# cemlyn007/ale-libtorch-ppo

Measured on AMD Instinct MI355X. Metric: env steps/sec (whole node), Breakout 84x84x4, higher is better.
Workload: dtype bf16

## Files before the change

### ale-libtorch-ppo_amd/csrc/gemm_launch.hip

```cpp
#include "common.hpp"
#include "gemm.hpp"
#include "gemm_pipe.hpp"
#include <algorithm>
#include <cstdlib>

namespace aleppo {

static int tune(const char *name, int dflt) {
  const char *e = std::getenv(name);
  return e ? std::atoi(e) : dflt;
}
static inline dim3 grid2(long M, int BM, long N, int BN, int Z = 1) {
  return dim3((unsigned)((M + BM - 1) / BM), (unsigned)((N + BN - 1) / BN), (unsigned)Z);
}

template <class T, bool IDX = false>
static void conv1_fwd_t(hipStream_t s, const uint32_t *obs, SampleMap map, const void *W1, const float *b1, void *a1,
                        long ns) {
  if constexpr (!IDX)
    if (map.idx)
      return conv1_fwd_t<T, true>(s, obs, map, W1, b1, a1, ns);
  using AL = ConvGatherLoader<T, uint8_t, 400, 20, 4, 84, 4, 8, IDX>;
  using BL = DenseLoader<T>;
  using EP = EpiBiasAct<T, true>;
  const long M = ns * 400;
  typename AL::P ap{reinterpret_cast<const uint8_t *>(obs), map.TP, map.s1 * 4, map.s0 * 4, map.base * 4, map.n0, map.idx};
  typename BL::P bp{static_cast<const T *>(W1), 256, 0};
  typename EP::P ep{static_cast<T *>(a1), b1, 32, 1.0f / 255.0f};
  hipLaunchKernelGGL((gemm_nt_kernel<T, AL, BL, EP, 128, 32, 4, 1>), grid2(M, 128, 32, 32), dim3(256), 0, s, ap, bp,
                     ep, (int)M, 32, 256);
}
template <class T>
static void conv2_fwd_t(hipStream_t s, const void *a1, const void *W2, const float *b2, void *a2, long ns) {
  using AL = ConvGatherLoader<T, T, 81, 9, 2, 20, 32, 4>;
  using BL = DenseLoader<T>;
  using EP = EpiBiasAct<T, true>;
  const long M = ns * 81;
  typename AL::P ap{static_cast<const T *>(a1), 1, 400 * 32, 0, 0, 0};
  typename BL::P bp{static_cast<const T *>(W2), 512, 0};
  typename EP::P ep{static_cast<T *>(a2), b2, 64, 1.0f};
  hipLaunchKernelGGL((gemm_nt_kernel<T, AL, BL, EP, 128, 64, 2, 2>), grid2(M, 128, 64, 64), dim3(256), 0, s, ap, bp,
                     ep, (int)M, 64, 512);
}
template <class T>
static void conv3_fwd_t(hipStream_t s, const void *a2, const void *W3, const float *b3, void *a3, long ns) {
  using AL = ConvGatherLoader<T, T, 49, 7, 1, 9, 64, 3>;
  using BL = DenseLoader<T>;
  using EP = EpiBiasAct<T, true>;
  const long M = ns * 49;
  typename AL::P ap{static_cast<const T *>(a2), 1, 81 * 64, 0, 0, 0};
  typename BL::P bp{static_cast<const T *>(W3), 576, 0};
  typename EP::P ep{static_cast<T *>(a3), b3, 64, 1.0f};
  hipLaunchKernelGGL((gemm_nt_kernel<T, AL, BL, EP, 128, 64, 2, 2>), grid2(M, 128, 64, 64), dim3(256), 0, s, ap, bp,
                     ep, (int)M, 64, 576);
}

static int pipe_cus() {
  static int n = 0;
  if (!n) {
    int dev = 0;
    hipDeviceProp_t p;
    if (hipGetDevice(&dev) == hipSuccess && hipGetDeviceProperties(&p, dev) == hipSuccess)
      n = p.multiProcessorCount;
    if (n <= 0)
      n = 256;
  }
  return n;
}
template <int MODE, int NST> static void launch_pipe(hipStream_t s, const PipeParams &P) {
  static bool once = false;
  constexpr size_t sm = gemm_pipe_smem<MODE, NST>();
  static_assert(sm <= 160 * 1024, "LDS budget");
  if (!once) {
    (void)hipFuncSetAttribute(reinterpret_cast<const void *>(gemm_pipe_kernel<MODE, NST>),
                              hipFuncAttributeMaxDynamicSharedMemorySize, (int)sm);
    once = true;
  }
  const int cus = pipe_cus() / 8 * 8, rounds = (P.njobs + cus - 1) / cus;
  const int grid = P.njobs >= cus / 4 ? std::min(cus, ((P.njobs + rounds - 1) / rounds + 7) / 8 * 8) : std::min(P.njobs, cus);
  hipLaunchKernelGGL((gemm_pipe_kernel<MODE, NST>), dim3(grid), dim3(PIPE_THREADS), sm, s, P);
}
static bool fc_dma() {
  static const bool v = tune("ALEPPO_FC_DMA", 1) != 0;
  return v;
}
static bool tn_xcd() {
  static const bool v = tune("ALEPPO_TN_XCD", 1) != 0;
  return v;
}
static bool use_pipe() { return tuning().fc_pipe; }
static int fc_fwd_pipe(hipStream_t s, const void *a3, const void *Wfc, const float *bfc, float *h, long ns, int H,
                       int max_parts) {
  const int tm = (int)((ns + 127) / 128), tn = (H + 127) / 128, tiles = tm * tn, cus = pipe_cus();
  int best = 1;
  double best_t = 1e30;
  for (int sp = 1; sp <= max_parts; ++sp) {
    const double t = (double)((tiles * sp + cus - 1) / cus) / sp + 0.02 * sp;
    if (t < best_t - 1e-9) {
      best_t = t;
      best = sp;
    }
  }
  PipeParams P{};
  P.A = static_cast<const bf16 *>(a3);
  P.lda = FC_IN;
  P.B = static_cast<const bf16 *>(Wfc);
  P.ldb = FC_IN;
  P.M = (int)ns;
  P.N = H;
  P.tiles_m = tm;
  P.tiles_n = tn;
  P.nstages = FC_IN / 64;
  P.splits = best;
  P.njobs = tiles * best;
  P.out_f32 = h;
  P.bias = bfc;
  launch_pipe<0, 4>(s, P);
  return best;
}
static void fc_dgrad_pipe(hipStream_t s, const void *dh, const void *WfcT, const void *a3, void *dz3, long ns, int H) {
  PipeParams P{};
  P.A = static_cast<const bf16 *>(dh);
  P.lda = H;
  P.B = static_cast<const bf16 *>(WfcT);
  P.ldb = H;
  P.M = (int)ns;
  P.N = FC_IN;
  P.tiles_m = (int)((ns + 127) / 128);
  P.tiles_n = (FC_IN + 127) / 128;
  P.nstages = H / 64;
  P.splits = 1;
  P.njobs = P.tiles_m * P.tiles_n;
  P.out_bf16 = static_cast<bf16 *>(dz3);
  P.gate = static_cast<const bf16 *>(a3);
  launch_pipe<1, 4>(s, P);
}
template <class T>
static void fc_fwd_t(hipStream_t s, const void *a3, const void *Wfc, const float *bfc, float *h, long ns, int H) {
  using AL = DenseLoader<T>;
  using BL = DenseLoader<T>;
  using EP = EpiBiasAct<float, false>;
  typename AL::P ap{static_cast<const T *>(a3), FC_IN, 0};
  typename BL::P bp{static_cast<const T *>(Wfc), FC_IN, 0};
  typename EP::P ep{h, bfc, H, 1.0f};
  if (ns <= 256)
    hipLaunchKernelGGL((gemm_nt_kernel<T, AL, BL, EP, 32, 32, 2, 2>), grid2(ns, 32, H, 32), dim3(256), 0, s, ap, bp,
                       ep, (int)ns, H, FC_IN);
  else if (fc_dma() && FC_IN % Atom<T>::KT == 0) {
    static const int v = tune("ALEPPO_FC_FWD_TILE", 1);
    const T *a = static_cast<const T *>(a3), *b = static_cast<const T *>(Wfc);
    if (v == 3 && FC_IN % (2 * Atom<T>::KT) == 0)
      hipLaunchKernelGGL((gemm_nt_dma_kernel<T, EP, 64, 64, 2, 2, 16>), grid2(ns, 64, H, 64), dim3(256), 0, s, a, FC_IN,
                         b, FC_IN, ep, (int)ns, H, FC_IN);
    else if (v == 4 && FC_IN % (2 * Atom<T>::KT) == 0)
      hipLaunchKernelGGL((gemm_nt_dma_kernel<T, EP, 128, 64, 2, 2, 16>), grid2(ns, 128, H, 64), dim3(256), 0, s, a,
                         FC_IN, b, FC_IN, ep, (int)ns, H, FC_IN);
    else if (v == 1)
      hipLaunchKernelGGL((gemm_nt_dma_kernel<T, EP, 64, 64, 2, 2>), grid2(ns, 64, H, 64), dim3(256), 0, s, a, FC_IN, b,
                         FC_IN, ep, (int)ns, H, FC_IN);
    else if (v == 2)
      hipLaunchKernelGGL((gemm_nt_dma_kernel<T, EP, 128, 128, 2, 2>), grid2(ns, 128, H, 128), dim3(256), 0, s, a,
                         FC_IN, b, FC_IN, ep, (int)ns, H, FC_IN);
    else
      hipLaunchKernelGGL((gemm_nt_dma_kernel<T, EP, 128, 64, 2, 2>), grid2(ns, 128, H, 64), dim3(256), 0, s, a, FC_IN,
                         b, FC_IN, ep, (int)ns, H, FC_IN);
  } else {
    static const int v = tune("ALEPPO_FC_FWD_TILE", 1);
    if (v == 1)
      hipLaunchKernelGGL((gemm_nt_kernel<T, AL, BL, EP, 64, 64, 2, 2>), grid2(ns, 64, H, 64), dim3(256), 0, s, ap, bp,
                         ep, (int)ns, H, FC_IN);
    else if (v == 2)
      hipLaunchKernelGGL((gemm_nt_kernel<T, AL, BL, EP, 128, 128, 2, 2>), grid2(ns, 128, H, 128), dim3(256), 0, s, ap,
                         bp, ep, (int)ns, H, FC_IN);
    else if (v == 3)
      hipLaunchKernelGGL((gemm_nt_kernel<T, AL, BL, EP, 64, 128, 2, 2>), grid2(ns, 64, H, 128), dim3(256), 0, s, ap,
                         bp, ep, (int)ns, H, FC_IN);
    else
      hipLaunchKernelGGL((gemm_nt_kernel<T, AL, BL, EP, 128, 64, 2, 2>), grid2(ns, 128, H, 64), dim3(256), 0, s, ap,
                         bp, ep, (int)ns, H, FC_IN);
  }
}

template <class T> static void fc_fwd_splitk_t(hipStream_t s, const void *a3, const void *Wfc, float *hpart, long ns, int H) {
  using AL = DenseLoader<T>;
  using BL = DenseLoader<T>;
  using EP = EpiPartial;
  constexpr int KC = FC_IN / FC_SPLITS;
  typename AL::P ap{static_cast<const T *>(a3), FC_IN, KC};
  typename BL::P bp{static_cast<const T *>(Wfc), FC_IN, KC};
  typename EP::P ep{hpart, H, ns * (long)H};
  hipLaunchKernelGGL((gemm_nt_kernel<T, AL, BL, EP, 32, 32, 2, 2>), grid2(ns, 32, H, 32, FC_SPLITS), dim3(256), 0, s,
                     ap, bp, ep, (int)ns, H, KC);
}
__global__ __launch_bounds__(256) void fc_act_kernel(const bf16 *__restrict__ a3, const bf16 *__restrict__ Wfc,
                                                     float *__restrict__ hpart, int M, int N) {
  constexpr int KC = FC_IN / FC_SPLITS, KS = KC / 32, VPR = KC / 8;
  constexpr int ROWV = VPR + 1;
  constexpr int NV = 32 * VPR / 256;
  __shared__ u32x4 sA[32 * ROWV], sB[32 * ROWV];
  const int tid = threadIdx.x, lane = tid & 63, wave = tid >> 6, fr = lane & 15, fg = lane >> 4;
  const int wm = wave >> 1, wn = wave & 1, z = blockIdx.z;
  const int m0 = blockIdx.x * 32, n0 = blockIdx.y * 32;
  u32x4 ra[NV], rb[NV];
#pragma unroll
  for (int i = 0; i < NV; ++i) {
    const int v = tid + 256 * i, r = v / VPR, c = v - r * VPR;
    ra[i] = *reinterpret_cast<const u32x4 *>(a3 + (long)min(m0 + r, M - 1) * FC_IN + z * KC + c * 8);
    rb[i] = *reinterpret_cast<const u32x4 *>(Wfc + (long)min(n0 + r, N - 1) * FC_IN + z * KC + c * 8);
  }
#pragma unroll
  for (int i = 0; i < NV; ++i) {
    const int v = tid + 256 * i, r = v / VPR, c = v - r * VPR;
    sA[r * ROWV + c] = ra[i];
    sB[r * ROWV + c] = rb[i];
  }
  __syncthreads();
  f32x4 acc = {0.f, 0.f, 0.f, 0.f};
#pragma unroll
  for (int ks = 0; ks < KS; ++ks)
    Atom<bf16>::mma(sA[(wm * 16 + fr) * ROWV + ks * 4 + fg], sB[(wn * 16 + fr) * ROWV + ks * 4 + fg], acc);
  float *out = hpart + (long)z * M * N;
  const int nn = n0 + wn * 16 + fr;
#pragma unroll
  for (int r = 0; r < 4; ++r) {
    const int mm = m0 + wm * 16 + fg * 4 + r;
    if (mm < M && nn < N)
      out[(long)mm * N + nn] = acc[r];
  }
}
void fc_fwd_splitk(hipStream_t s, int prec, const void *a3, const void *Wfc, float *hpart, long ns, int H) {
  static const bool latency_form = tune("ALEPPO_FC_ACT_LATENCY", 1) != 0;
  if (prec == ALEPPO_BF16 && latency_form)
    hipLaunchKernelGGL(fc_act_kernel, grid2(ns, 32, H, 32, FC_SPLITS), dim3(256), 0, s, static_cast<const bf16 *>(a3),
                       static_cast<const bf16 *>(Wfc), hpart, (int)ns, H);
  else if (prec == ALEPPO_BF16)
    fc_fwd_splitk_t<bf16>(s, a3, Wfc, hpart, ns, H);
  else
    fc_fwd_splitk_t<float>(s, a3, Wfc, hpart, ns, H);
}

template <class T>
static void fc_dgrad_t(hipStream_t s, const void *dh, const void *WfcT, const void *a3, void *dz3, long ns, int H) {
  using AL = DenseLoader<T>;
  using BL = DenseLoader<T>;
  using EP = EpiReluMask<T, 0>;
  typename AL::P ap{static_cast<const T *>(dh), H, 0};
  typename BL::P bp{static_cast<const T *>(WfcT), H, 0};
  typename EP::P ep{static_cast<T *>(dz3), static_cast<const T *>(a3), FC_IN, 0};
  static const int v = tune("ALEPPO_FC_DGRAD_TILE", 1);
  if (fc_dma() && H % Atom<T>::KT == 0) {
    const T *a = static_cast<const T *>(dh), *b = static_cast<const T *>(WfcT);
    if (v == 3)
      hipLaunchKernelGGL((gemm_nt_dma_kernel<T, EP, 64, 64, 2, 2, 16>), grid2(ns, 64, FC_IN, 64), dim3(256), 0, s, a, H,
                         b, H, ep, (int)ns, FC_IN, H);
    else if (v == 4)
      hipLaunchKernelGGL((gemm_nt_dma_kernel<T, EP, 128, 64, 2, 2, 16>), grid2(ns, 128, FC_IN, 64), dim3(256), 0, s, a,
                         H, b, H, ep, (int)ns, FC_IN, H);
    else if (v == 2)
      hipLaunchKernelGGL((gemm_nt_dma_kernel<T, EP, 128, 128, 2, 2>), grid2(ns, 128, FC_IN, 128), dim3(256), 0, s, a,
                         H, b, H, ep, (int)ns, FC_IN, H);
    else if (v == 0)
      hipLaunchKernelGGL((gemm_nt_dma_kernel<T, EP, 128, 64, 2, 2>), grid2(ns, 128, FC_IN, 64), dim3(256), 0, s, a, H,
                         b, H, ep, (int)ns, FC_IN, H);
    else
      hipLaunchKernelGGL((gemm_nt_dma_kernel<T, EP, 64, 64, 2, 2>), grid2(ns, 64, FC_IN, 64), dim3(256), 0, s, a, H, b,
                         H, ep, (int)ns, FC_IN, H);
    return;
  }
  if (v == 1)
    hipLaunchKernelGGL((gemm_nt_kernel<T, AL, BL, EP, 64, 64, 2, 2>), grid2(ns, 64, FC_IN, 64), dim3(256), 0, s, ap, bp,
                       ep, (int)ns, FC_IN, H);
  else if (v == 2)
    hipLaunchKernelGGL((gemm_nt_kernel<T, AL, BL, EP, 128, 128, 2, 2>), grid2(ns, 128, FC_IN, 128), dim3(256), 0, s,
                       ap, bp, ep, (int)ns, FC_IN, H);
  else
    hipLaunchKernelGGL((gemm_nt_kernel<T, AL, BL, EP, 128, 64, 2, 2>), grid2(ns, 128, FC_IN, 64), dim3(256), 0, s, ap,
                       bp, ep, (int)ns, FC_IN, H);
}
template <class T>
static void conv3_dgrad_t(hipStream_t s, const void *dz3, const void *W3d, const void *a2, void *dz2, long ns) {
  using AL = DgradGatherLoader<T, 9, 9, 7, 7, 64, 3>;
  using BL = DenseLoader<T>;
  using EP = EpiReluMask<T, 0>;
  const long M = ns * 81;
  typename AL::P ap{static_cast<const T *>(dz3)};
  typename BL::P bp{static_cast<const T *>(W3d), 576, 0};
  typename EP::P ep{static_cast<T *>(dz2), static_cast<const T *>(a2), 64, 0};
  hipLaunchKernelGGL((gemm_nt_kernel<T, AL, BL, EP, 128, 64, 2, 2>), grid2(M, 128, 64, 64), dim3(256), 0, s, ap, bp,
                     ep, (int)M, 64, 576);
}
template <class T>
static void conv2_dgrad_t(hipStream_t s, const void *dz2, const void *W2d, const void *a1, void *dz1, long ns) {
  using AL = DgradGatherLoader<T, 10, 10, 9, 9, 64, 2>;
  using BL = DenseLoader<T>;
  using EP = EpiReluMask<T, 1>;
  const long M = ns * 100;
  typename AL::P ap{static_cast<const T *>(dz2)};
  typename BL::P bp{static_cast<const T *>(W2d), 256, 32 * 256};
  typename EP::P ep{static_cast<T *>(dz1), static_cast<const T *>(a1), 32, 0};
  hipLaunchKernelGGL((gemm_nt_kernel<T, AL, BL, EP, 128, 32, 4, 1>), grid2(M, 128, 32, 32, 4), dim3(256), 0, s, ap,
                     bp, ep, (int)M, 32, 256);
}

static inline int pick_slices(long Ktot, int KP, int tiles_mn, int maxS) {
  long S = 512 / tiles_mn;
  const long cap = Ktot / (2L * KP);
  if (S > cap)
    S = cap;
  if (S > maxS)
    S = maxS;
  if (S < 1)
    S = 1;
  return (int)S;
}
static inline int chunk_for(long Ktot, int S, int KP) {
  long c = (Ktot + S - 1) / S;
  c = (c + KP - 1) / KP * KP;
  return (int)c;
}

static int fc_wgrad_split_max() { return tune("ALEPPO_FC_WGRAD_SPLIT", 2); }

template <class T> static int fc_wgrad_t(hipStream_t s, const void *dh, const void *a3, float *sw, float *sb, long ns, int H) {
  using AL = DenseLoader<T>;
  using BL = DenseLoader<T>;
  constexpr int KP = Atom<T>::KT;
  static const int v = tune("ALEPPO_FC_WGRAD_TILE", 0);
  static const int smax = fc_wgrad_split_max();
  const int S = (int)std::max<long>(1, std::min<long>(std::min(smax, MAXS_FC), ns / (4 * KP)));
  const int kc = chunk_for(ns, S, KP);
  typename AL::P ap{static_cast<const T *>(dh), H, 0};
  typename BL::P bp{static_cast<const T *>(a3), FC_IN, 0};
  auto swz = [&](const dim3 &g) { return ((g.x * g.y * S) % 8 == 0 && tn_xcd()) ? (int)(g.x | (g.y << 12)) : 0; };
  auto grid = [&](const dim3 &g, int xsw) { return xsw ? dim3(g.x * g.y * S) : dim3(g.x, g.y, S); };
  if (v == 1) {
    const dim3 g = grid2(H, 64, FC_IN, 64);
    const int xsw = swz(g);
    hipLaunchKernelGGL((gemm_tn_kernel<T, AL, BL, 64, 64, 2, 2, true>), grid(g, xsw), dim3(256), 0, s, ap, bp, sw,
                       sb, H, FC_IN, (int)ns, kc, 1.0f, xsw);
  } else if (v == 2) {
    const dim3 g = grid2(H, 128, FC_IN, 64);
    const int xsw = swz(g);
    hipLaunchKernelGGL((gemm_tn_kernel<T, AL, BL, 128, 64, 2, 2, true>), grid(g, xsw), dim3(256), 0, s, ap, bp,
                       sw, sb, H, FC_IN, (int)ns, kc, 1.0f, xsw);
  } else {
    const dim3 g = grid2(H, 64, FC_IN, 128);
    const int xsw = swz(g);
    hipLaunchKernelGGL((gemm_tn_kernel<T, AL, BL, 64, 128, 2, 2, true>), grid(g, xsw), dim3(256), 0, s, ap, bp,
                       sw, sb, H, FC_IN, (int)ns, kc, 1.0f, xsw);
  }
  return S;
}
template <class T> static int conv3_wgrad_t(hipStream_t s, const void *dz3, const void *a2, float *sw, float *sb, long ns) {
  using AL = DenseLoader<T>;
  using BL = ConvGatherLoader<T, T, 49, 7, 1, 9, 64, 3>;
  constexpr int KP = Atom<T>::KT;
  const long K = ns * 49;
  const dim3 g = grid2(64, 64, 576, 64);
  const int S = pick_slices(K, KP, g.x * g.y, MAXS_C3);
  const int kc = chunk_for(K, S, KP);
  typename AL::P ap{static_cast<const T *>(dz3), 64, 0};
  typename BL::P bp{static_cast<const T *>(a2), 1, 81 * 64, 0, 0, 0};
  hipLaunchKernelGGL((gemm_tn_kernel<T, AL, BL, 64, 64, 2, 2, true>), dim3(g.x, g.y, S), dim3(256), 0, s, ap, bp, sw,
                     sb, 64, 576, (int)K, kc, 1.0f, 0);
  return S;
}
template <class T> static int conv2_wgrad_t(hipStream_t s, const void *dz2, const void *a1, float *sw, float *sb, long ns) {
  using AL = DenseLoader<T>;
  using BL = ConvGatherLoader<T, T, 81, 9, 2, 20, 32, 4>;
  constexpr int KP = Atom<T>::KT;
  const long K = ns * 81;
  const dim3 g = grid2(64, 64, 512, 128);
  const int S = pick_slices(K, KP, g.x * g.y, MAXS_C2);
  const int kc = chunk_for(K, S, KP);
  typename AL::P ap{static_cast<const T *>(dz2), 64, 0};
  typename BL::P bp{static_cast<const T *>(a1), 1, 400 * 32, 0, 0, 0};
  hipLaunchKernelGGL((gemm_tn_kernel<T, AL, BL, 64, 128, 2, 2, true>), dim3(g.x, g.y, S), dim3(256), 0, s, ap, bp, sw,
                     sb, 64, 512, (int)K, kc, 1.0f, 0);
  return S;
}
template <class T, bool IDX = false>
static int conv1_wgrad_t(hipStream_t s, const void *dz1, const uint32_t *obs, SampleMap map, float *sw, float *sb,
                         long ns) {
  if constexpr (!IDX)
    if (map.idx)
      return conv1_wgrad_t<T, true>(s, dz1, obs, map, sw, sb, ns);
  using AL = DenseLoader<T>;
  using BL = ConvGatherLoader<T, uint8_t, 400, 20, 4, 84, 4, 8, IDX>;
  constexpr int KP = Atom<T>::KT;
  const long K = ns * 400;
  const dim3 g = grid2(32, 32, 256, 128);
  const int S = pick_slices(K, KP, g.x * g.y, MAXS_C1);
  const int kc = chunk_for(K, S, KP);
  typename AL::P ap{static_cast<const T *>(dz1), 32, 0};
  typename BL::P bp{reinterpret_cast<const uint8_t *>(obs), map.TP, map.s1 * 4, map.s0 * 4, map.base * 4, map.n0, map.idx};
  hipLaunchKernelGGL((gemm_tn_kernel<T, AL, BL, 32, 128, 1, 4, true>), dim3(g.x, g.y, S), dim3(256), 0, s, ap, bp, sw,
                     sb, 32, 256, (int)K, kc, 1.0f / 255.0f, 0);
  return S;
}

#define DISPATCH(prec, call_f32, call_bf16)                                                                            \
  do {                                                                                                                 \
    if ((prec) == ALEPPO_BF16) {                                                                                       \
      call_bf16;                                                                                                       \
    } else {                                                                                                           \
      call_f32;                                                                                                        \
    }                                                                                                                  \
  } while (0)

void conv1_fwd(hipStream_t s, int prec, const uint32_t *obs, SampleMap map, const void *W1, const float *b1, void *a1,
               long ns) {
  if (prec == ALEPPO_BF16 && use_patch_kernels())
    return patch_conv1_fwd(s, obs, map, W1, b1, a1, ns);
  DISPATCH(prec, conv1_fwd_t<float>(s, obs, map, W1, b1, a1, ns), conv1_fwd_t<bf16>(s, obs, map, W1, b1, a1, ns));
}
void conv2_fwd(hipStream_t s, int prec, const void *a1, const void *W2, const float *b2, void *a2, long ns) {
  if (prec == ALEPPO_BF16 && use_patch_kernels())
    return patch_conv2_fwd(s, a1, W2, b2, a2, ns);
  DISPATCH(prec, conv2_fwd_t<float>(s, a1, W2, b2, a2, ns), conv2_fwd_t<bf16>(s, a1, W2, b2, a2, ns));
}
void conv3_fwd(hipStream_t s, int prec, const void *a2, const void *W3, const float *b3, void *a3, long ns) {
  if (prec == ALEPPO_BF16 && use_patch_kernels())
    return patch_conv3_fwd(s, a2, W3, b3, a3, ns);
  DISPATCH(prec, conv3_fwd_t<float>(s, a2, W3, b3, a3, ns), conv3_fwd_t<bf16>(s, a2, W3, b3, a3, ns));
}
int fc_fwd(hipStream_t s, int prec, const void *a3, const void *Wfc, const float *bfc, float *h, long ns, int H,
           int max_parts) {
  if (prec == ALEPPO_BF16 && ns > 256 && H % 64 == 0 && H >= 64 && use_pipe())
    return fc_fwd_pipe(s, a3, Wfc, bfc, h, ns, H, std::max(1, std::min(max_parts, FC_FWD_MAX_PARTS)));
  DISPATCH(prec, fc_fwd_t<float>(s, a3, Wfc, bfc, h, ns, H), fc_fwd_t<bf16>(s, a3, Wfc, bfc, h, ns, H));
  return 1;
}
void fc_dgrad(hipStream_t s, int prec, const void *dh, const void *WfcT, const void *a3, void *dz3, long ns, int H) {
  if (prec == ALEPPO_BF16 && ns > 256 && H % 64 == 0 && H >= 4 * 64 && use_pipe())
    return fc_dgrad_pipe(s, dh, WfcT, a3, dz3, ns, H);
  DISPATCH(prec, fc_dgrad_t<float>(s, dh, WfcT, a3, dz3, ns, H), fc_dgrad_t<bf16>(s, dh, WfcT, a3, dz3, ns, H));
}
void conv3_dgrad(hipStream_t s, int prec, const void *dz3, const void *W3d, const void *a2, void *dz2, long ns) {
  if (prec == ALEPPO_BF16 && use_patch_kernels())
    return patch_conv3_dgrad(s, dz3, W3d, a2, dz2, ns);
  DISPATCH(prec, conv3_dgrad_t<float>(s, dz3, W3d, a2, dz2, ns), conv3_dgrad_t<bf16>(s, dz3, W3d, a2, dz2, ns));
}
void conv2_dgrad(hipStream_t s, int prec, const void *dz2, const void *W2d, const void *a1, void *dz1, long ns) {
  if (prec == ALEPPO_BF16 && use_patch_kernels())
    return patch_conv2_dgrad(s, dz2, W2d, a1, dz1, ns);
  DISPATCH(prec, conv2_dgrad_t<float>(s, dz2, W2d, a1, dz1, ns), conv2_dgrad_t<bf16>(s, dz2, W2d, a1, dz1, ns));
}
int fc_wgrad_slices(int prec, long ns) {
  static const int smax = fc_wgrad_split_max();
  const int KP = prec == ALEPPO_BF16 ? Atom<bf16>::KT : Atom<float>::KT;
  return (int)std::max<long>(1, std::min<long>(std::min(smax, MAXS_FC), ns / (4 * KP)));
}
int fc_wgrad(hipStream_t s, int prec, const void *dh, const void *a3, float *sw, float *sb, long ns, int H) {
  if (prec == ALEPPO_BF16)
    return fc_wgrad_t<bf16>(s, dh, a3, sw, sb, ns, H);
  return fc_wgrad_t<float>(s, dh, a3, sw, sb, ns, H);
}
int conv3_wgrad(hipStream_t s, int prec, const void *dz3, const void *a2, float *sw, float *sb, long ns) {
  if (prec == ALEPPO_BF16 && use_patch_kernels())
    return patch_conv3_wgrad(s, dz3, a2, sw, sb, ns);
  if (prec == ALEPPO_BF16)
    return conv3_wgrad_t<bf16>(s, dz3, a2, sw, sb, ns);
  return conv3_wgrad_t<float>(s, dz3, a2, sw, sb, ns);
}
int conv2_wgrad(hipStream_t s, int prec, const void *dz2, const void *a1, float *sw, float *sb, long ns) {
  if (prec == ALEPPO_BF16 && use_patch_kernels())
    return patch_conv2_wgrad(s, dz2, a1, sw, sb, ns);
  if (prec == ALEPPO_BF16)
    return conv2_wgrad_t<bf16>(s, dz2, a1, sw, sb, ns);
  return conv2_wgrad_t<float>(s, dz2, a1, sw, sb, ns);
}
int conv1_wgrad(hipStream_t s, int prec, const void *dz1, const uint32_t *obs, SampleMap map, float *sw, float *sb,
                long ns) {
  if (prec == ALEPPO_BF16 && use_patch_kernels())
    return patch_conv1_wgrad(s, dz1, obs, map, sw, sb, ns);
  if (prec == ALEPPO_BF16)
    return conv1_wgrad_t<bf16>(s, dz1, obs, map, sw, sb, ns);
  return conv1_wgrad_t<float>(s, dz1, obs, map, sw, sb, ns);
}

}
```

### ale-libtorch-ppo_amd/csrc/gemm_pipe.hpp

```cpp
#pragma once
#include "gemm.hpp"

namespace aleppo {

struct PipeParams {
  const bf16 *A;
  long lda;
  const bf16 *B;
  long ldb;
  int M, N;
  int tiles_m, tiles_n;
  int nstages;
  int splits;
  int njobs;
  float *out_f32;
  const float *bias;
  bf16 *out_bf16;
  const bf16 *gate;
};

template <int N> __device__ __forceinline__ void wait_vm() { asm volatile("s_waitcnt vmcnt(%0)" ::"n"(N) : "memory"); }
constexpr int PIPE_STAGE_CHUNKS = 2048;
template <int MODE, int NST> constexpr size_t gemm_pipe_smem() {
  return (size_t)(NST * PIPE_STAGE_CHUNKS + (MODE == 1 ? 128 * 16 : 0)) * 16;
}

struct PipeFrags {
  u32x4 a[2][4], b[2][2];
};

constexpr int PIPE_THREADS = 768;
template <int MODE, int NST> __global__ __launch_bounds__(PIPE_THREADS) void gemm_pipe_kernel(PipeParams P) {
  constexpr int NL = 4, PPL = 32 / NL;
  static_assert(NST >= 3, "ring depth");
  extern __shared__ __attribute__((aligned(16))) uint8_t smem[];
  u32x4 *ring = reinterpret_cast<u32x4 *>(smem);
  u32x4 *etile = ring + NST * PIPE_STAGE_CHUNKS;
  typedef __attribute__((address_space(1))) const void *gptr;
  typedef __attribute__((address_space(3))) void *lptr;

  const int tid = threadIdx.x, lane = tid & 63, wave = tid >> 6;
  const bool loader = wave >= 8;
  const int lw = wave - 8;
  const int fr = lane & 15, fg = lane >> 4;
  const int wm = (wave & 7) >> 2, wn = wave & 3;
  const int eslot = tid & 15, er0 = (tid & 511) >> 4;

  const bool grouped = gridDim.x % 8 == 0;
  const bool xmap = grouped && P.tiles_m % 8 == 0, pmap = grouped && !xmap;
  const int xcd = (int)blockIdx.x % 8;
  const int tmx = xmap ? P.tiles_m / 8 : P.tiles_m;
  const int npairs = P.tiles_n * P.splits;
  const int pairs_g = pmap ? (npairs - xcd + 7) / 8 : npairs;
  const int jobs_g = tmx * pairs_g;
  const int wg_l = grouped ? (int)blockIdx.x / 8 : (int)blockIdx.x;
  const int nwg_l = grouped ? (int)gridDim.x / 8 : (int)gridDim.x;
  const int tm_base = xmap ? xcd * tmx : 0;
  const int nj = (jobs_g - wg_l + nwg_l - 1) / nwg_l;
  if (nj <= 0)
    return;
  struct Job {
    int m0, n0, slice, ks0, nks;
  };
  auto decode = [&](int ord) {
    const int j = wg_l + ord * nwg_l;
    int slice, tm, tn;
    if (pmap) {
      const int pr = xcd + 8 * (j / tmx);
      tm = j % tmx;
      slice = pr % P.splits;
      tn = pr / P.splits;
    } else {
      slice = j % P.splits;
      const int t = j / P.splits;
      tm = tm_base + t % tmx;
      tn = t / tmx;
    }
    const int ks0 = (int)((long)slice * P.nstages / P.splits), ks1 = (int)((long)(slice + 1) * P.nstages / P.splits);
    return Job{tm * 128, tn * 128, slice, ks0, ks1 - ks0};
  };
  int G = 0;
#pragma nounroll
  for (int o = 0; o < nj; ++o)
    G += decode(o).nks;

  int cord = 0, ck = 0;
  Job cjob = decode(0);
  if (loader) {
    int pord = 0, pk = 0, pissued = 0, pbuf = 0;
    Job pjob = cjob;
    const bf16 *ps[PPL];
    auto set_src = [&]() {
#pragma unroll
      for (int q = 0; q < PPL; ++q) {
        const int wp = lw + NL * q, c = (wp & 15) * 64 + lane, r = c >> 3, sw = ((c & 7) ^ (r & 7)) * 8;
        ps[q] = wp < 16 ? P.A + (long)min(pjob.m0 + r, P.M - 1) * P.lda + (long)pjob.ks0 * 64 + sw
                        : P.B + (long)min(pjob.n0 + r, P.N - 1) * P.ldb + (long)pjob.ks0 * 64 + sw;
      }
    };
    set_src();
    auto issue = [&]() {
#pragma unroll
      for (int q = 0; q < PPL; ++q)
        __builtin_amdgcn_global_load_lds((gptr)(ps[q] + (long)pk * 64),
                                         (lptr)(ring + pbuf * PIPE_STAGE_CHUNKS + (lw + NL * q) * 64), 16, 0, 0);
      pbuf = pbuf + 1 == NST ? 0 : pbuf + 1;
      ++pissued;
      if (++pk == pjob.nks && ++pord < nj) {
        pjob = decode(pord);
        pk = 0;
        set_src();
      }
    };
    auto wait_stage_batches = [&](int batches) {
      switch (batches) {
      case 0: wait_vm<0>(); break;
      case 1: wait_vm<PPL>(); break;
      case 2: wait_vm<2 * PPL>(); break;
      default: wait_vm<(3 * PPL < 63 ? 3 * PPL : 63)>(); break;
      }
    };
#pragma nounroll
    for (int i = 0; i < NST && pissued < G; ++i)
      issue();
    wait_stage_batches(min(NST - 1, G - 1));
    __builtin_amdgcn_s_barrier();
#pragma nounroll
    for (int g = 0; g < G; ++g) {
      if (g + 1 < G)
        wait_stage_batches(min(NST - 2, G - 2 - g));
      __builtin_amdgcn_s_barrier();
      if (pissued < G)
        issue();
      if (++ck == cjob.nks) {
        if constexpr (MODE == 1) {
          __builtin_amdgcn_s_barrier();
          __builtin_amdgcn_s_barrier();
        }
        ck = 0;
        if (++cord < nj)
          cjob = decode(cord);
      }
    }
    return;
  }

  int cbuf = 0;
  auto read_a = [&](PipeFrags &f, int buf, int kc, int i) {
    const int r = wm * 64 + i * 16 + fr;
    f.a[kc][i] = ring[buf * PIPE_STAGE_CHUNKS + r * 8 + ((kc * 4 + fg) ^ (r & 7))];
  };
  auto read_b = [&](PipeFrags &f, int buf, int kc, int j) {
    const int r = wn * 32 + j * 16 + fr;
    f.b[kc][j] = ring[buf * PIPE_STAGE_CHUNKS + 1024 + r * 8 + ((kc * 4 + fg) ^ (r & 7))];
  };
  f32x4 acc[4][2];
  auto zero_acc = [&]() {
#pragma unroll
    for (int i = 0; i < 4; ++i)
#pragma unroll
      for (int j = 0; j < 2; ++j)
        acc[i][j] = f32x4{0.f, 0.f, 0.f, 0.f};
  };
  zero_acc();
  PipeFrags F0, F1;
  {
    __builtin_amdgcn_s_barrier();
#pragma unroll
    for (int kc = 0; kc < 2; ++kc) {
#pragma unroll
      for (int j = 0; j < 2; ++j)
        read_b(F0, 0, kc, j);
#pragma unroll
      for (int i = 0; i < 4; ++i)
        read_a(F0, 0, kc, i);
    }
    cbuf = 1;
  }

  auto stage = [&](int g, PipeFrags &cur, PipeFrags &nxt) {
    const bool has_next = g + 1 < G;
    asm volatile("s_waitcnt lgkmcnt(0)" ::: "memory");
    __builtin_amdgcn_s_barrier();
    __builtin_amdgcn_sched_barrier(0);
#pragma unroll
    for (int q = 0; q < 4; ++q) {
#pragma unroll
      for (int u = 0; u < 4; ++u) {
        const int kc = q >> 1, i = (q & 1) * 2 + (u >> 1), j = u & 1;
        Atom<bf16>::mma(cur.b[kc][j], cur.a[kc][i], acc[i][j]);
      }
      __builtin_amdgcn_sched_barrier(0);
      if (has_next) {
        const int kc = q >> 1, h = q & 1;
        read_b(nxt, cbuf, kc, h);
        read_a(nxt, cbuf, kc, 2 * h);
        read_a(nxt, cbuf, kc, 2 * h + 1);
      }
      __builtin_amdgcn_sched_barrier(0);
    }
    if (has_next)
      cbuf = cbuf + 1 == NST ? 0 : cbuf + 1;
    if constexpr (MODE == 1) {
      if (ck == 0) {
#pragma unroll
        for (int i = 0; i < 4; ++i) {
          const int r = er0 + 32 * i;
          const bf16 *src =
              P.gate + (long)min(cjob.m0 + r, P.M - 1) * P.N + min(cjob.n0 + ((eslot ^ (r & 15)) * 8), P.N - 8);
          __builtin_amdgcn_global_load_lds((gptr)src, (lptr)(etile + wave * 64 + 512 * i), 16, 0, 0);
        }
      }
    }
    if (++ck == cjob.nks) {
      const int mrow = cjob.m0 + wm * 64 + fr, ncol = cjob.n0 + wn * 32 + fg * 4;
      if constexpr (MODE == 0) {
        {
          float *out = P.out_f32 + (long)cjob.slice * P.M * P.N;
#pragma unroll
          for (int j = 0; j < 2; ++j) {
            const int n = ncol + j * 16;
            f32x4 b = {0.f, 0.f, 0.f, 0.f};
            if (cjob.slice == 0 && n < P.N)
              b = *reinterpret_cast<const f32x4 *>(P.bias + n);
#pragma unroll
            for (int i = 0; i < 4; ++i) {
              const int m = mrow + i * 16;
              if (m < P.M && n < P.N)
                *reinterpret_cast<f32x4 *>(out + (long)m * P.N + n) = acc[i][j] + b;
            }
          }
        }
      } else {
        wait_vm<0>();
        __builtin_amdgcn_s_barrier();
        {
          uint8_t *eb = reinterpret_cast<uint8_t *>(etile);
#pragma unroll
          for (int i = 0; i < 4; ++i)
#pragma unroll
            for (int j = 0; j < 2; ++j) {
              const int r = wm * 64 + i * 16 + fr, c = wn * 32 + j * 16 + fg * 4;
              u32x2 *p = reinterpret_cast<u32x2 *>(eb + r * 256 + (((c >> 3) ^ (r & 15)) * 16) + (c & 7) * 2);
              const u32x2 gt = *p;
              auto on = [](uint32_t w, int hi) {
                const uint32_t h = hi ? (w >> 16) : (w & 0xFFFFu);
                return (h & 0x7FFFu) != 0 && (h & 0x8000u) == 0;
              };
              const float v0 = on(gt[0], 0) ? acc[i][j][0] : 0.f, v1 = on(gt[0], 1) ? acc[i][j][1] : 0.f;
              const float v2 = on(gt[1], 0) ? acc[i][j][2] : 0.f, v3 = on(gt[1], 1) ? acc[i][j][3] : 0.f;
              typedef __attribute__((ext_vector_type(2))) __bf16 bf16x2;
              const bf16x2 lo = {(bf16)v0, (bf16)v1}, hi = {(bf16)v2, (bf16)v3};
              *p = u32x2{__builtin_bit_cast(uint32_t, lo), __builtin_bit_cast(uint32_t, hi)};
            }
          asm volatile("s_waitcnt lgkmcnt(0)" ::: "memory");
        }
        __builtin_amdgcn_s_barrier();
        {
#pragma unroll
          for (int i = 0; i < 4; ++i) {
            const int r = er0 + 32 * i, m = cjob.m0 + r, n = cjob.n0 + ((eslot ^ (r & 15)) * 8);
            const u32x4 v = etile[r * 16 + eslot];
            if (m < P.M && n < P.N)
              *reinterpret_cast<u32x4 *>(P.out_bf16 + (long)m * P.N + n) = v;
          }
        }
      }
      zero_acc();
      ck = 0;
      if (++cord < nj)
        cjob = decode(cord);
    }
  };

#pragma nounroll
  for (int g = 0; g < G; g += 2) {
    stage(g, F0, F1);
    if (g + 1 < G)
      stage(g + 1, F1, F0);
  }
}

}
```

Measured before the change: 1.516 million.

## Route bf16 FC weight-gradient through pipelined DMA GEMM with transposed LDS reads

Adds a MODE 2 path to the persistent pipelined GEMM kernel for the FC weight gradient (dh^T · a3). It loads K-major tiles with global-to-LDS DMA and uses ds_read_tr16 transposed LDS reads to build MFMA fragments. A separate small kernel reduces the bias gradient per split slice. The launch grid is also adjusted per XCD when the M-tile count is not a multiple of 8. The goal is to replace the generic wgrad kernel with the overlapped load/compute pipeline. In exchange it adds an extra bias kernel launch and scalar fp32 stores in the epilogue.

```diff
diff --git a/ale-libtorch-ppo_amd/csrc/gemm_launch.hip b/ale-libtorch-ppo_amd/csrc/gemm_launch.hip
--- a/ale-libtorch-ppo_amd/csrc/gemm_launch.hip
+++ b/ale-libtorch-ppo_amd/csrc/gemm_launch.hip
@@ -77,7 +77,11 @@
     once = true;
   }
   const int cus = pipe_cus() / 8 * 8, rounds = (P.njobs + cus - 1) / cus;
-  const int grid = P.njobs >= cus / 4 ? std::min(cus, ((P.njobs + rounds - 1) / rounds + 7) / 8 * 8) : std::min(P.njobs, cus);
+  int grid = P.njobs >= cus / 4 ? std::min(cus, ((P.njobs + rounds - 1) / rounds + 7) / 8 * 8) : std::min(P.njobs, cus);
+  if (MODE == 2 && P.tiles_m % 8 != 0 && P.njobs >= cus / 4) {
+    const int per_xcd = P.tiles_m * ((P.tiles_n * P.splits + 7) / 8), r = (per_xcd + cus / 8 - 1) / (cus / 8);
+    grid = 8 * ((per_xcd + r - 1) / r);
+  }
   hipLaunchKernelGGL((gemm_pipe_kernel<MODE, NST>), dim3(grid), dim3(PIPE_THREADS), sm, s, P);
 }
 static bool fc_dma() {
@@ -134,6 +138,52 @@
   P.out_bf16 = static_cast<bf16 *>(dz3);
   P.gate = static_cast<const bf16 *>(a3);
   launch_pipe<1, 4>(s, P);
+}
+__global__ __launch_bounds__(256) void fc_bias_grad_kernel(const bf16 *__restrict__ dh, float *__restrict__ sb, int H,
+                                                           int nstages, int cs) {
+  __shared__ float part[16][16];
+  const int c = threadIdx.x & 15, t = threadIdx.x >> 4, m = blockIdx.x * 16 + c, z = blockIdx.y;
+  const int g0 = z * cs, g1 = min(nstages, g0 + cs);
+  float bsum = 0.f;
+  for (int gb = g0; gb < g1; gb += 16) {
+    float st = 0.f;
+    if (gb + t < g1 && m < H) {
+      const bf16 *p = dh + (long)(gb + t) * 64 * H + m;
+      float v[64];
+#pragma unroll
+      for (int r = 0; r < 64; ++r)
+        v[r] = (float)p[(long)r * H];
+#pragma unroll
+      for (int r = 0; r < 64; ++r)
+        st += v[r];
+    }
+    part[t][c] = st;
+    __syncthreads();
+    if (t == 0)
+      for (int u = 0; u < 16 && gb + u < g1; ++u)
+        bsum += part[u][c];
+    __syncthreads();
+  }
+  if (t == 0 && m < H)
+    sb[(long)z * H + m] = bsum;
+}
+static void fc_wgrad_pipe(hipStream_t s, const void *dh, const void *a3, float *sw, float *sb, long ns, int H, int S) {
+  PipeParams P{};
+  P.A = static_cast<const bf16 *>(dh);
+  P.lda = H;
+  P.B = static_cast<const bf16 *>(a3);
+  P.ldb = FC_IN;
+  P.M = H;
+  P.N = FC_IN;
+  P.tiles_m = (H + 127) / 128;
+  P.tiles_n = (FC_IN + 127) / 128;
+  P.nstages = (int)(ns / 64);
+  P.splits = S;
+  P.njobs = P.tiles_m * P.tiles_n * S;
+  P.out_f32 = sw;
+  hipLaunchKernelGGL(fc_bias_grad_kernel, dim3((unsigned)((H + 15) / 16), (unsigned)S), dim3(256), 0, s, P.A, sb, H,
+                     P.nstages, (P.nstages + S - 1) / S);
+  launch_pipe<2, 4>(s, P);
 }
 template <class T>
 static void fc_fwd_t(hipStream_t s, const void *a3, const void *Wfc, const float *bfc, float *h, long ns, int H) {
@@ -452,6 +502,11 @@
   return (int)std::max<long>(1, std::min<long>(std::min(smax, MAXS_FC), ns / (4 * KP)));
 }
 int fc_wgrad(hipStream_t s, int prec, const void *dh, const void *a3, float *sw, float *sb, long ns, int H) {
+  const int S = fc_wgrad_slices(prec, ns);
+  if (prec == ALEPPO_BF16 && ns > 256 && ns % 64 == 0 && ns / 64 >= 4 * S && H % 64 == 0 && use_pipe()) {
+    fc_wgrad_pipe(s, dh, a3, sw, sb, ns, H, S);
+    return S;
+  }
   if (prec == ALEPPO_BF16)
     return fc_wgrad_t<bf16>(s, dh, a3, sw, sb, ns, H);
   return fc_wgrad_t<float>(s, dh, a3, sw, sb, ns, H);
diff --git a/ale-libtorch-ppo_amd/csrc/gemm_pipe.hpp b/ale-libtorch-ppo_amd/csrc/gemm_pipe.hpp
--- a/ale-libtorch-ppo_amd/csrc/gemm_pipe.hpp
+++ b/ale-libtorch-ppo_amd/csrc/gemm_pipe.hpp
@@ -19,6 +19,8 @@
   const bf16 *gate;
 };
 
+__device__ __forceinline__ int wg_swz(int r) { return ((r & 3) << 2) | ((r >> 1) & 2); }
+
 template <int N> __device__ __forceinline__ void wait_vm() { asm volatile("s_waitcnt vmcnt(%0)" ::"n"(N) : "memory"); }
 constexpr int PIPE_STAGE_CHUNKS = 2048;
 template <int MODE, int NST> constexpr size_t gemm_pipe_smem() {
@@ -76,7 +78,9 @@
       tm = tm_base + t % tmx;
       tn = t / tmx;
     }
-    const int ks0 = (int)((long)slice * P.nstages / P.splits), ks1 = (int)((long)(slice + 1) * P.nstages / P.splits);
+    const int cs = (P.nstages + P.splits - 1) / P.splits;
+    const int ks0 = MODE == 2 ? slice * cs : (int)((long)slice * P.nstages / P.splits);
+    const int ks1 = MODE == 2 ? min(P.nstages, ks0 + cs) : (int)((long)(slice + 1) * P.nstages / P.splits);
     return Job{tm * 128, tn * 128, slice, ks0, ks1 - ks0};
   };
   int G = 0;
@@ -93,16 +97,25 @@
     auto set_src = [&]() {
 #pragma unroll
       for (int q = 0; q < PPL; ++q) {
-        const int wp = lw + NL * q, c = (wp & 15) * 64 + lane, r = c >> 3, sw = ((c & 7) ^ (r & 7)) * 8;
-        ps[q] = wp < 16 ? P.A + (long)min(pjob.m0 + r, P.M - 1) * P.lda + (long)pjob.ks0 * 64 + sw
-                        : P.B + (long)min(pjob.n0 + r, P.N - 1) * P.ldb + (long)pjob.ks0 * 64 + sw;
+        const int wp = lw + NL * q;
+        if constexpr (MODE == 2) {
+          const int c = (wp & 15) * 64 + lane, r = c >> 4, ch = (c & 15) ^ wg_swz(r);
+          const long kr = (long)pjob.ks0 * 64 + r;
+          ps[q] = wp < 16 ? P.A + kr * P.lda + min(pjob.m0 + ch * 8, P.M - 8)
+                          : P.B + kr * P.ldb + min(pjob.n0 + ch * 8, P.N - 8);
+        } else {
+          const int c = (wp & 15) * 64 + lane, r = c >> 3, sw = ((c & 7) ^ (r & 7)) * 8;
+          ps[q] = wp < 16 ? P.A + (long)min(pjob.m0 + r, P.M - 1) * P.lda + (long)pjob.ks0 * 64 + sw
+                          : P.B + (long)min(pjob.n0 + r, P.N - 1) * P.ldb + (long)pjob.ks0 * 64 + sw;
+        }
       }
     };
+    auto kstep = [&](int q) -> long { return MODE == 2 ? 64L * (q < NL ? P.lda : P.ldb) : 64L; };
     set_src();
     auto issue = [&]() {
 #pragma unroll
       for (int q = 0; q < PPL; ++q)
-        __builtin_amdgcn_global_load_lds((gptr)(ps[q] + (long)pk * 64),
+        __builtin_amdgcn_global_load_lds((gptr)(ps[q] + pk * kstep(q)),
                                          (lptr)(ring + pbuf * PIPE_STAGE_CHUNKS + (lw + NL * q) * 64), 16, 0, 0);
       pbuf = pbuf + 1 == NST ? 0 : pbuf + 1;
       ++pissued;
@@ -146,13 +159,34 @@
   }
 
   int cbuf = 0;
+  auto read_tr = [&](int buf, int img, int kc, int c0) {
+    typedef short s16x4 __attribute__((ext_vector_type(4)));
+    typedef __attribute__((address_space(3))) s16x4 *tptr;
+    const int q = fr >> 2, p = fr & 3;
+    u32x2 h2[2];
+#pragma unroll
+    for (int h = 0; h < 2; ++h) {
+      const int r = kc * 32 + h * 16 + fg * 4 + q, slot = (c0 + (p >> 1)) ^ wg_swz(r);
+      uint8_t *a = reinterpret_cast<uint8_t *>(ring + buf * PIPE_STAGE_CHUNKS + img * 1024 + r * 16 + slot) + 8 * (p & 1);
+      h2[h] = __builtin_bit_cast(u32x2, __builtin_amdgcn_ds_read_tr16_b64_v4i16((tptr)a));
+    }
+    return u32x4{h2[0][0], h2[0][1], h2[1][0], h2[1][1]};
+  };
   auto read_a = [&](PipeFrags &f, int buf, int kc, int i) {
-    const int r = wm * 64 + i * 16 + fr;
-    f.a[kc][i] = ring[buf * PIPE_STAGE_CHUNKS + r * 8 + ((kc * 4 + fg) ^ (r & 7))];
+    if constexpr (MODE == 2) {
+      f.a[kc][i] = read_tr(buf, 0, kc, wm * 8 + i * 2);
+    } else {
+      const int r = wm * 64 + i * 16 + fr;
+      f.a[kc][i] = ring[buf * PIPE_STAGE_CHUNKS + r * 8 + ((kc * 4 + fg) ^ (r & 7))];
+    }
   };
   auto read_b = [&](PipeFrags &f, int buf, int kc, int j) {
-    const int r = wn * 32 + j * 16 + fr;
-    f.b[kc][j] = ring[buf * PIPE_STAGE_CHUNKS + 1024 + r * 8 + ((kc * 4 + fg) ^ (r & 7))];
+    if constexpr (MODE == 2) {
+      f.b[kc][j] = read_tr(buf, 1, kc, wn * 4 + j * 2);
+    } else {
+      const int r = wn * 32 + j * 16 + fr;
+      f.b[kc][j] = ring[buf * PIPE_STAGE_CHUNKS + 1024 + r * 8 + ((kc * 4 + fg) ^ (r & 7))];
+    }
   };
   f32x4 acc[4][2];
   auto zero_acc = [&]() {
@@ -188,7 +222,10 @@
 #pragma unroll
       for (int u = 0; u < 4; ++u) {
         const int kc = q >> 1, i = (q & 1) * 2 + (u >> 1), j = u & 1;
-        Atom<bf16>::mma(cur.b[kc][j], cur.a[kc][i], acc[i][j]);
+        if constexpr (MODE == 2)
+          Atom<bf16>::mma(cur.a[kc][i], cur.b[kc][j], acc[i][j]);
+        else
+          Atom<bf16>::mma(cur.b[kc][j], cur.a[kc][i], acc[i][j]);
       }
       __builtin_amdgcn_sched_barrier(0);
       if (has_next) {
@@ -214,7 +251,21 @@
     }
     if (++ck == cjob.nks) {
       const int mrow = cjob.m0 + wm * 64 + fr, ncol = cjob.n0 + wn * 32 + fg * 4;
-      if constexpr (MODE == 0) {
+      if constexpr (MODE == 2) {
+        float *out = P.out_f32 + (long)cjob.slice * P.M * P.N;
+#pragma unroll
+        for (int i = 0; i < 4; ++i)
+#pragma unroll
+          for (int r = 0; r < 4; ++r) {
+            const int m = cjob.m0 + wm * 64 + i * 16 + fg * 4 + r;
+#pragma unroll
+            for (int j = 0; j < 2; ++j) {
+              const int n = cjob.n0 + wn * 32 + j * 16 + fr;
+              if (m < P.M && n < P.N)
+                out[(long)m * P.N + n] = acc[i][j][r];
+            }
+          }
+      } else if constexpr (MODE == 0) {
         {
           float *out = P.out_f32 + (long)cjob.slice * P.M * P.N;
 #pragma unroll
```

Result: no change. 1.530 million, median of 6 (+0.9%).
